# fgiral000/gencast-flax-nnx

Measured on AMD Instinct MI355X. Metric: denoiser-calls/sec, higher is better.
Workload: dtype f16x3 (every product = 3 fp16 MFMAs on hi/lo-split f32 operands: 22-bit products, f32 accumulate; f32 storage); 1 GPU; nano-GenCast DPM-Solver++2S 20-step sample, 2.5deg grid (73x144), 1 ensemble member per GPU, batch 1; dead_call_skipped=True, grid_nodes=10512, mesh_nodes=2562, latent=256, layers=16, heads=4, ffw_hidden=2048, c_in=262, c_out=82, k_hop=8, parallelism=ensemble-dp1, broadcast=none, rccl_ranks=0, precision=f16x3, library_built_from_this_tree=True, launcher=single

## Files before the change

gencast-flax-nnx_amd/csrc/gc_api.hip:

```cpp
#include <dlfcn.h>

#include "gc_handle.h"

using namespace gci;

namespace {

void protect_pending_noise(gc_handle* h) {
  if (h->guard_pending && h->d_noise == h->last_noise) std::swap(h->d_noise, h->d_noise_alt);
}

int check_ready(gc_handle* h) {
  if (!h) return GC_ERR_INVALID_ARGUMENT;
  if (!h->finalized) return fail(h, GC_ERR_STATE, "gc_finalize has not been called");
  return GC_OK;
}

struct Rccl {
  void* lib = nullptr;
  ncclResult_t (*GetUniqueId)(ncclUniqueId*) = nullptr;
  ncclResult_t (*CommInitRank)(ncclComm_t*, int, ncclUniqueId, int) = nullptr;
  ncclResult_t (*CommDestroy)(ncclComm_t) = nullptr;
  ncclResult_t (*CommCount)(const ncclComm_t, int*) = nullptr;
  ncclResult_t (*CommUserRank)(const ncclComm_t, int*) = nullptr;
// ... 67 lines not shown
  if (!out || cap < 16 || device_id < 0 || device_id >= gc_device_count()) return GC_ERR_INVALID_ARGUMENT;
  out[0] = 0;
  return hipDeviceGetPCIBusId(out, (int)cap, device_id) == hipSuccess ? GC_OK : GC_ERR_HIP;
}

const char* gc_last_error(const gc_handle* h) { return h ? h->err.c_str() : g_create_error.c_str(); }

static void read_switches(gc_handle* h) {
  auto is = [](const char* name, const char* value) { const char* v = std::getenv(name); return v && std::string(v) == value; };
  auto off = [](const char* name) { const char* v = std::getenv(name); return v && *v && std::atoi(v) == 0; };
  auto on = [](const char* name) { const char* v = std::getenv(name); return v && *v == '1'; };
  h->f16x3 = !is("GC_PRECISION", "f32");
  h->use_graphs = !is("GC_TUNE_GRAPH", "0");
  h->m2g_fuse_sum = !off("GC_TUNE_M2G_FUSE_SUM");
  h->embed_cache = !off("GC_TUNE_EMBED_CACHE");
  h->attn_items = !off("GC_TUNE_ATTN_ITEMS");
  h->mlp_pair = !off("GC_TUNE_MLP_PAIR");
  h->a16 = !off("GC_TUNE_A16");
  h->graph_serialize = on("GC_TUNE_GRAPH_SERIALIZE");
  h->graph_verbose = on("GC_TUNE_GRAPH_VERBOSE");
}

int gc_create(const gc_config* cfg, int device_id, gc_handle** out) {
  return guarded(nullptr, [&]() -> int {
  if (!cfg || !out) { g_create_error = "null argument"; return GC_ERR_INVALID_ARGUMENT; }
  *out = nullptr;
  const gc_config& c = *cfg;
  auto bad = [&](const char* m) { g_create_error = m; return GC_ERR_INVALID_ARGUMENT; };
  if (c.latent_size <= 0 || c.d_model <= 0 || c.num_heads <= 0 || c.ffw_hidden <= 0 ||
      c.num_layers < 0 || c.c_in <= 0 || c.c_out <= 0 || c.batch <= 0)
// ... 683 lines not shown

int gc_get_counter(gc_handle* h, const char* name, int64_t* value) {
  return guarded(h, [&]() -> int {
  if (!h) return GC_ERR_INVALID_ARGUMENT;
  if (!name || !value) return fail(h, GC_ERR_INVALID_ARGUMENT, "null argument");
  const std::string n(name);
  if (n == "range_fallbacks") *value = h->range_fallbacks;
  else if (n == "static_embedding_fallbacks") *value = h->static_embedding_fallbacks;
  else if (n == "launches_per_call") *value = h->launches_last_call;
  else if (n == "weights_f16_unsafe") *value = h->weights_f16_unsafe ? 1 : 0;
  else if (n == "fp16_storage") *value = h->last_route.st16 ? 1 : 0;
  else if (n == "split_edge") *value = h->split_edge ? 1 : 0;
  else if (n == "attention_items") *value = h->last_route.att_items;
  else if (n == "m2g_fused_sum") *value = h->last_route.m2g_fused ? 1 : 0;
  else if (n == "embed_cache") *value = h->embed_cache_samples;
  else if (n == "graph_replays") *value = h->graph_replays;
  else if (n == "graph_captures") *value = h->graph_captures;
  else if (n == "loss_evaluations") *value = h->loss_evaluations;
  else if (n == "loss_device_us") *value = h->loss_device_us;
  else if (n == "ens_scores") *value = h->ens_scores;
  else if (n == "ens_score_device_us") *value = h->ens_score_device_us;
  else if (n == "ens_invalid_points") *value = h->ens_invalid_points;
  else if (n == "spec_calls") *value = h->spec_calls;
  else if (n == "spec_device_us") *value = h->spec_device_us;
  else if (n == "spec_invalid_columns") *value = h->spec_invalid_columns;
  else if (n == "ens_event_calls") *value = h->evt_calls;
  else if (n == "ens_event_device_us") *value = h->evt_device_us;
  else if (n == "ens_event_invalid_points") *value = h->evt_invalid_points;
  else if (n == "ens_derive_calls") *value = h->drv_calls;
  else if (n == "ens_derive_device_us") *value = h->drv_device_us;
// ... 374 lines not shown
  });
}

int gc_debug_fetch(gc_handle* h, const char* name, float* out, int64_t capacity, int64_t* rows,
                   int64_t* cols) {
  return guarded(h, [&]() -> int {
  int rc = check_ready(h);
  if (rc) return rc;
  if (!name || !rows || !cols) return fail(h, GC_ERR_INVALID_ARGUMENT, "null argument");
  const gc_config& c = h->cfg;
  const gc::HostGraph& g = h->hg;
  const int64_t B = c.batch, L = c.latent_size;
  struct Ent { const char* n; const float* p; int64_t items; int64_t w; int mesh; int batched; int act; };
  const Ent table[] = {
      {"cond", h->d_condvec, 1, gc::kCondDim, 0, 1, 0},
      {"g0", h->d_g0, g.G, L, 0, 1, 1},        {"m0", h->d_m0, g.M, L, 1, 1, 1},
      {"e1", h->d_e1, g.E1, L, 0, 1, 1},       {"agg1", h->d_agg1, g.M, L, 1, 1, 1},
      {"m1", h->d_x, g.M, L, 1, 1, 1},         {"x", h->d_x, g.M, L, 1, 1, 1},
      {"g1", h->d_g1, g.G, L, 0, 1, 1},        {"qkv", h->d_qkv, g.M, 3 * L, 1, 1, 0},
      {"att", h->d_att, g.M, L, 1, 1, 1},      {"m2", h->d_m2, g.M, L, 1, 1, 1},
      {"h", h->d_h, g.M, L, 1, 1, 1},
      {"f1", h->d_f1, g.E2, L, 0, 1, 1},       {"agg2", h->d_agg2, g.G, L, 0, 1, 1},
      {"g2", h->d_g2, g.G, L, 0, 1, 1},        {"y", h->d_y, g.G, c.c_out, 0, 1, 0},
      {"m0_hat", h->d_m0_hat, g.M, L, 1, 0, 0}, {"e0_hat", h->d_e0_hat, g.E1, L, 0, 0, 0},
      {"f0_hat", h->d_f0_hat, g.E2, L, 0, 0, 0},
  };
  if (!std::strncmp(name, "cond:", 5)) {
    auto it = h->cond_sites.find(name + 5);
    if (it == h->cond_sites.end()) return fail(h, GC_ERR_INVALID_ARGUMENT, std::string("unknown conditioning site: ") + (name + 5));
    const int off = it->second.first, w = it->second.second;
    *rows = B;
// ... 123 lines not shown
```

gencast-flax-nnx_amd/csrc/gc_forward.hip:

```cpp
#include "gc_handle.h"

namespace gci {

template <class To, class From>
static const To& a16_view(const From& v) {
  static_assert(sizeof(To) == sizeof(From), "argument struct mismatch between the two kernel builds");
  return reinterpret_cast<const To&>(v);
}

Route make_route(const gc_handle* h) {
  const int D = h->cfg.d_model, F = h->cfg.ffw_hidden;
  Route r;
  r.f16 = h->f16x3 && !h->weights_f16_unsafe && !h->in_fallback;
  r.x32 = !r.f16 && h->f32_ws;
  const bool streams = r.f16 || r.x32;
  r.ffw_slabs = streams ? h->ffw_fused_slabs : 0;
  r.st16 = h->feat16 && h->a16 && r.f16 && D % 128 == 0 && D <= 512 &&
           (h->ffw_fused_slabs > 0 || (F % 128 == 0 && (F / h->ffw2_splits) % 128 == 0));
  r.v2 = r.f16 && r.ws(3 * D, D, 1);
  r.att_items = (h->att_n_items > 0 && r.ws(3 * D, D, 1) && h->attn_splits == 1 && D <= 512) ? h->att_n_items : 0;
  r.fuse_row = streams && D % 128 == 0 && D <= 512;
  r.node_ws = r.f16;
  r.split_edge = h->split_edge;
  r.try_pair = h->mlp_pair && h->hidden_layers == 1;
  r.m2g_fused = h->m2g_fuse_sum && h->hg.m2g_tri && h->hidden_layers == 1 && streams;
  r.embed_cache = h->embed_cache_live && h->embed_cache_ready && !h->feat16 && h->hidden_layers == 1 && streams;
  return r;
}

static gc::Segment seg(const float* ptr, const int* index, const float* affine, int width, int ld, int bcast) {
  gc::Segment s;
  s.ptr = ptr; s.index = index; s.affine = affine; s.width = width; s.ld = ld; s.bcast = bcast;
  return s;
}

struct MlpCall {
  gc::Segment seg[3] = {};
  gc::AddTerm add[2] = {};
  int nseg = 0, nadd = 0, rows = 0, B = 1, ldo = 0;
  bool ln = true, cond = true;
  const float* residual = nullptr;
  float* out = nullptr;
  bool round_out = true;
  bool seg0_f32 = false, out_f32 = false;
  bool tri = false;
  MlpCall& segments(std::initializer_list<gc::Segment> l) { for (const auto& s : l) seg[nseg++] = s; return *this; }
  MlpCall& add_terms(std::initializer_list<gc::AddTerm> l) { for (const auto& t : l) add[nadd++] = t; return *this; }
};
static MlpCall mlp_call(std::initializer_list<gc::Segment> segs, int rows, int B, float* out, int ldo,
                        const float* residual = nullptr) {
  MlpCall c;
  c.rows = rows; c.B = B; c.out = out; c.ldo = ldo; c.residual = residual;
  return c.segments(segs);
}

static int build_mlp_args(gc_handle* h, const DevMlp& w, const MlpCall& c, gc::MlpArgs* out_args) {
  const Route& r = h->route;
  gc::MlpArgs& a = *out_args;
  a = gc::MlpArgs{};
  a.nseg = c.nseg; a.nadd = c.nadd;
  std::copy(c.seg, c.seg + c.nseg, a.seg);
  std::copy(c.add, c.add + c.nadd, a.add);
  a.rows = c.rows; a.B = c.B; a.hidden = h->cfg.latent_size;
  a.f16 = r.f16 ? 1 : 0;
  const Weight& w1 = c.nadd ? w.w1e : w.w1;
  a.w1t = pick(w1, r, Form::Staged); a.ldw1 = w1.ld; a.b1 = w.b1;
  a.w2t = pick(w.w2, r, Form::Staged); a.b2 = w.b2;
  if (r.f16 || r.x32) {
    a.w1f = pick(w1, r, Form::Streaming); a.k1f = w1.kf;
    a.w2f = pick(w.w2, r, Form::Streaming); a.ones = h->d_ones; a.zeros = h->d_zeros;
    a.f32w = r.x32 ? 1 : 0;
  }
  a.n_out = w.n_out; a.n_out_pad = w.n_out_pad; a.do_ln = c.ln ? 1 : 0;
  a.cond = (c.cond && w.cond_off >= 0) ? (h->cond_cur ? h->cond_cur : h->d_cond) + w.cond_off : nullptr;
  a.cond_stride = h->cond_total;
  a.residual = c.residual; a.out = c.out; a.ldo = c.ldo;
  a.round16 = h->feat16 ? 1 : 0;
  a.round_out = (h->feat16 && c.round_out) ? 1 : 0;
  a.a16 = r.st16 ? 1 : 0;
  a.seg0_f32 = c.seg0_f32 ? 1 : 0;
// ... 123 lines not shown
  ga.round16 = 0;
  ga.out_f32 = 1;
  if (r.node_ws) {
    ga.wt = pick(w, r, Form::Streaming); ga.a16 = r.st16 ? 1 : 0;
    return enqueue_gemm_ws(h, gc::KC_GEMM_NODE, ga, pick_ws_mt(rows, L, 1), 1, 0);
  }
  ga.wt = pick(w, r, Form::Staged);
  return launch(h, gc::KC_GEMM_NODE, [&] { return gc::launch_gemm(h->stream, gc::KC_GEMM_NODE, ga, 1, 0, r.f16); });
}
static int edge_node_products(gc_handle* h, const DevMlp& w, const float* senders, int snd_rows, float* snd_out,
                              const float* receivers, int rcv_rows, float* rcv_out) {
  if (int rc = node_gemm(h, senders, snd_rows, w.w1snd, snd_out)) return rc;
  return node_gemm(h, receivers, rcv_rows, w.w1rcv, rcv_out);
}

static MlpCall edge_call(gc_handle* h, const float* e_hat, const float* e_affine, int E, const int* snd, const int* rcv,
                         const float* nsnd, const float* nrcv, const float* psnd, const float* prcv, float* out) {
  const int B = h->cfg.batch, L = h->cfg.latent_size;
  MlpCall c = mlp_call({seg(e_hat, nullptr, e_affine, L, L, 1)}, E * B, B, out, L);
  c.seg0_f32 = true;
  if (h->route.split_edge) c.add_terms({{psnd, snd}, {prcv, rcv}});
  else c.segments({seg(nsnd, snd, nullptr, L, L, 0), seg(nrcv, rcv, nullptr, L, L, 0)});
  return c;
}

int run_m2g_edge(gc_handle* h, const float* cond, bool fused) {
  MlpCall c = edge_call(h, h->d_f0_hat, cond + h->m2g_embed_edge.cond_off, h->hg.E2, h->d_m2g_snd, h->d_m2g_rcv,
                        h->d_m2, h->d_g1, h->d_pm, h->d_pg, fused ? h->d_agg2 : h->d_f1);
  c.tri = fused;
  return run_mlp(h, h->m2g_edge, c);
// ... 11 lines not shown
  if (h->attn_splits > 1) ga->att_S = h->attn_splits;
  else ga->att_tiles = h->d_att_tiles;
}
static int mesh_gemm(gc_handle* h, int cls, const float* a, int lda, const Weight& w, int n, int k, int splits,
                     const float* bias, int act, float* out, int ldo, int epi, bool att_merge = false) {
  const Route& r = h->route;
  const bool ws = r.ws(n, k, splits);
  gc::GemmArgs ga = mesh_gemm_args(h, a, lda, ws);
  ga.wt = pick(w, r, ws ? Form::Streaming : Form::Staged); ga.ldw = k; ga.n = n; ga.k_slice = k / splits;
  ga.bias = bias; ga.act = act; ga.out = out; ga.ldo = ldo;
  if (att_merge) merge_attention_partials(h, &ga);
  if (ws) return enqueue_gemm_ws(h, cls, ga, att_merge ? 1 : pick_ws_mt(ga.rows, n, splits), splits, epi);
  return launch(h, cls, [&] { return gc::launch_gemm(h->stream, cls, ga, splits, epi, r.f16); });
}

int forward(gc_handle* h, float sigma_scalar, const float* cond_ready) {
  const gc_config& c = h->cfg;
  const gc::HostGraph& g = h->hg;
  const int B = c.batch, L = c.latent_size, D = c.d_model, F = c.ffw_hidden;
  hipStream_t s = h->stream;
  int rc;
  const float* cond = cond_ready ? cond_ready : h->d_cond;
  h->cond_cur = cond;
  const int cs = h->cond_total;
  const int64_t launches0 = h->launch_count;
  const Route& r = h->route = h->last_route = make_route(h);

  if (!cond_ready && (rc = launch(h, gc::KC_COND, [&] {
         return gc::launch_cond(s, sigma_scalar < 0 ? h->d_sigma : nullptr, sigma_scalar, B, h->d_nw0t,
                                h->d_nb0, h->d_nw1t, h->d_nb1, c.noise_num_frequencies, c.noise_hidden,
                                c.noise_base_period, h->d_wc_all, h->d_bc_all, cs, h->d_condvec,
                                h->d_cond);
       })))
    return rc;

  {
    MlpCall embed = r.embed_cache ? mlp_call({seg(h->d_xn, nullptr, nullptr, h->nwp, h->nwp, 0)}, g.G * B, B, h->d_g0, L)
                                  : mlp_call({seg(h->d_xp, nullptr, nullptr, h->kp, h->kp, 0)}, g.G * B, B, h->d_g0, L);
    embed.seg0_f32 = true;
    if (r.embed_cache) embed.add_terms({{h->d_pstat, nullptr}});
    if ((rc = run_mlp(h, r.embed_cache ? h->g2m_embed_grid_n : h->g2m_embed_grid, embed))) return rc;
  }
  if ((rc = launch(h, gc::KC_PACK, [&] {
         return gc::launch_affine_rows(s, h->d_m0_hat, cond + h->g2m_embed_mesh.cond_off, cs, g.M, B, L,
                                       h->d_m0, h->feat16, r.st16);
       })))
    return rc;
  const MlpCall edge = edge_call(h, h->d_e0_hat, cond + h->g2m_embed_edge.cond_off, g.E1, h->d_g2m_snd, h->d_g2m_rcv,
                                 h->d_g0, h->d_m0, h->d_pg, h->d_pm, h->d_e1);
  const MlpCall node = mlp_call({seg(h->d_g0, nullptr, nullptr, L, L, 0)}, g.G * B, B, h->d_g1, L, h->d_g0);
  gc::MlpArgs ea{}, na{};
  bool paired = false;
  if (r.try_pair) {
    if ((rc = build_mlp_args(h, h->g2m_edge, edge, &ea)) || (rc = build_mlp_args(h, h->g2m_grid, node, &na))) return rc;
    paired = gc::mlp_pair_supported(ea, na);
  }
  if (r.split_edge && (rc = edge_node_products(h, h->g2m_edge, h->d_g0, g.G * B, h->d_pg, h->d_m0, g.M * B, h->d_pm)))
    return rc;
  if ((rc = paired ? enqueue_mlp_pair(h, ea, na) : run_mlp(h, h->g2m_edge, edge))) return rc;
  if ((rc = launch(h, gc::KC_SEGSUM, [&] {
         return gc::launch_segsum(s, h->d_e1, h->d_g2m_ptr, h->d_g2m_eid, g.M, g.E1, B, L, h->d_agg1, h->feat16, r.st16,
                                  h->g2m_agg_norm);
       })))
    return rc;
  if ((rc = run_mlp(h, h->g2m_mesh, mlp_call({seg(h->d_m0, nullptr, nullptr, L, L, 0), seg(h->d_agg1, nullptr, nullptr, L, L, 0)},
                                             g.M * B, B, h->d_x, L, h->d_m0))))
    return rc;
  if (!paired && (rc = run_mlp(h, h->g2m_grid, node))) return rc;

  const int MB = g.M * B;
  const int n_layers = (h->debug_layer_limit >= 0 && h->debug_layer_limit < c.num_layers)
                           ? h->debug_layer_limit : c.num_layers;
  const float* pend_bias = nullptr;
  int pend_slabs = 0;
  auto rowop = [&](const float* bias, int slabs, int cond_off, float* hout) {
    return launch(h, gc::KC_ROWOP, [&] {
      return gc::launch_rowop(s, h->d_x, bias, h->d_part, slabs, MB, D, B, cond + cond_off, cs, hout, 0, h->feat16, r.st16);
    });
  };
  auto stop_here = [&](int i, int phase) { return h->debug_stop_layer == i && h->debug_stop_phase == phase; };
  const int* att_items = r.att_items ? h->d_att_items : nullptr;
  for (int i = 0; i < n_layers; ++i) {
// ... 108 lines not shown
```

gencast-flax-nnx_amd/csrc/gc_handle.h:

```cpp
#pragma once
#include <hip/hip_runtime.h>

#include <algorithm>
#include <array>
#include <cmath>
#include <cstdio>
#include <cstdlib>
#include <cstring>
#include <map>
#include <memory>
#include <mutex>
#include <string>
#include <vector>

#include <rccl/rccl.h>

#include "../../include/gencast_hip.h"
#include "../../include/gencast_hip_debug.h"
#include "gc_graph.h"
#include "gc_kernels.h"

namespace gci {

inline int round_up(int v, int m) { return (v + m - 1) / m * m; }

struct Route {
  bool f16 = false;
  bool x32 = false;
  bool st16 = false;
  int ffw_slabs = 0;
  bool v2 = false;
  int att_items = 0;
  bool fuse_row = false;
  bool node_ws = false;
  bool m2g_fused = false;
  bool split_edge = false;
  bool try_pair = false;
  bool embed_cache = false;
  bool ws(int n, int k, int splits) const { return (f16 || x32) && n % 128 == 0 && (k / splits) % 128 == 0; }
};

struct Weight {
  float* t = nullptr;
  float* s = nullptr;
  float* f = nullptr;
  float* x = nullptr;
  int ld = 0, kf = 0;
};
enum class Form { Staged, Streaming };
inline const float* pick(const Weight& w, const Route& r, Form form) {
  if (form == Form::Streaming) return r.x32 ? w.x : w.f;
  return r.f16 ? w.s : w.t;
}

struct DevMlp {
  Weight w1, w2;
  Weight w1e, w1snd, w1rcv;
  float *b1 = nullptr, *b2 = nullptr;
  int n_out = 0, n_out_pad = 0;
  int cond_off = -1;
  std::vector<DevMlp> pre;
};

struct DevLayer {
  Weight wqkv, wo, w1, w2;
  float *bo = nullptr, *b1 = nullptr, *b2 = nullptr;
  int cond_attn = -1, cond_ffw = -1;
};

struct BufferGroup {
  std::vector<void*> ptrs;
  explicit BufferGroup(std::vector<BufferGroup*>& of_handle) { of_handle.push_back(this); }
// ... 81 lines not shown
  float *d_feats = nullptr, *d_xp = nullptr, *d_g0 = nullptr, *d_g1 = nullptr, *d_m0 = nullptr,
        *d_x = nullptr, *d_e1 = nullptr, *d_agg1 = nullptr, *d_qkv = nullptr, *d_att = nullptr,
        *d_u = nullptr, *d_m2 = nullptr, *d_f1 = nullptr, *d_agg2 = nullptr, *d_g2 = nullptr,
        *d_y = nullptr, *d_h = nullptr, *d_part = nullptr, *d_apart_o = nullptr, *d_apart_ml = nullptr,
        *d_pg = nullptr, *d_pm = nullptr;
  bool mlp_pair = true;
  bool embed_cache = true;
  bool embed_cache_ready = false;
  bool embed_cache_live = false;
  int nwp = 0;
  float *d_xn = nullptr, *d_pstat = nullptr;
  float *w1st_t = nullptr, *w1st_s = nullptr;
  gci::DevMlp g2m_embed_grid_n;
  std::vector<int> h_slots;
  int64_t embed_cache_samples = 0;
  bool m2g_fuse_sum = true;
  float *d_ones = nullptr, *d_zeros = nullptr;
  int hidden_layers = 1;
  float* d_mlp_tmp[2] = {nullptr, nullptr};
  float *d_feats2 = nullptr, *d_ro_a = nullptr, *d_ro_b = nullptr, *d_ro_forc = nullptr;
  int *d_ro_kind = nullptr, *d_ro_src = nullptr, *d_ro_sidx = nullptr;
  int ro_nforc = -1, ro_forc_cap = 0;
  bool has_sample = false;
  int max_tile_chunks = 0;
  int ffw_fused_slabs = 0;
  void* d_kv16 = nullptr;
  bool f32_ws = true;
  bool split_edge = false;
  int attn_splits = 1, out_splits = 1, ffw2_splits = 1;
  gci::Route route;
// ... 170 lines not shown
  int reg_dev_M = 0;
  int* d_reg_plan = nullptr;
  double* d_reg_part = nullptr;
  unsigned* d_reg_hpart = nullptr;
  double* d_reg_sums = nullptr;
  unsigned long long* d_reg_hist = nullptr;
  gci::Bracket reg_time{events};
  int64_t reg_calls = 0, reg_device_us = 0, reg_invalid_points = 0;

  struct SampleGraph {
    std::vector<float> sigmas;
    int skip_dead = 1;
    const float* noise = nullptr;
    bool feat16 = false;
    gci::Route route;
    hipGraph_t graph = nullptr;
    hipGraphExec_t exec = nullptr, exec2 = nullptr;
    hipEvent_t done[2] = {nullptr, nullptr};
    int next = 0;
    int calls = 0;
    int64_t launches_per_call = 0, launches = 0;
    uint64_t last_use = 0;
  };
  bool use_graphs = true;
  std::vector<SampleGraph> sample_graphs;
  uint64_t graph_clock = 0;
  int64_t graph_replays = 0, graph_captures = 0;
  int debug_layer_limit = -1;
  int debug_stop_layer = -1, debug_stop_phase = -1;
  bool f16x3 = true;
// ... 112 lines not shown
  }
  try {
    (h ? h->err : g_create_error) = what;
  } catch (...) {
  }
  return GC_ERR_INTERNAL;
}

extern const char* const P_M2G;
void build_specs(gc_handle* h);
float f16_bits_to_f32(uint16_t h);
void free_weights(gc_handle* h);
int finalize_weights(gc_handle* h);
int build_embed_cache(gc_handle* h);
Route make_route(const gc_handle* h);
bool build_attention_items(const gc::HostGraph& g, std::vector<int>* items, std::vector<int>* tiles);
int run_m2g_edge(gc_handle* h, const float* cond, bool fused);
int forward(gc_handle* h, float sigma_scalar, const float* cond_ready = nullptr);
int compute_static_embeddings(gc_handle* h);
int guard_enqueue(gc_handle* h, const float* p, size_t n);
bool guard_tripped(gc_handle* h);
int noise_field(gc_handle* h, const float* base, float scale, float* out);
int run_sampler(gc_handle* h, const float* sigmas, int n, int skip_dead, gc_sample_stats* stats);
int resolve_guard(gc_handle* h);
void destroy_sample_graph(gc_handle::SampleGraph& g);
void drop_sample_graphs(gc_handle* h);
int loss_eval(gc_handle* h, int e, const float* sig, bool draw_noise, bool want_den);

}
```

gencast-flax-nnx_amd/csrc/gc_kernels.hip:

```cpp
#include "gc_kernels.h"

#include <algorithm>
#include <atomic>
#include <type_traits>

#include <math.h>
#include <stdlib.h>

#ifdef GC_TU_A16
#define GC_TU_NS gc_a16
#else
#define GC_TU_NS gc
#endif
namespace GC_TU_NS {
#ifdef GC_TU_A16
constexpr bool kTuA16 = true;
#else
constexpr bool kTuA16 = false;
#endif

#include "gc_dev_common.inc"


struct DynLdsOnce {
// ... 3443 lines not shown
__global__ __launch_bounds__(256) void gc_dpm_second_kernel(const float* __restrict__ y,
                                                             const float* __restrict__ xmid,
                                                             float c_out, float c_skip, float a_next,
                                                             size_t n, float* __restrict__ x, NoisyWrite nw) {
  for (size_t i = (size_t)blockIdx.x * 256 + threadIdx.x; i < n; i += (size_t)gridDim.x * 256) {
    const float md = y[i] * c_out + xmid[i] * c_skip;
    const float v = a_next * x[i] + (1.0f - a_next) * md;
    x[i] = v;
    if (nw.xp || nw.xn) put_noisy(nw, i, v);
  }
}

__global__ __launch_bounds__(256) void gc_affine_rows_kernel(const float* __restrict__ src,
                                                              const float* __restrict__ cond,
                                                              int cond_stride, size_t items, int B,
                                                              int w, float* __restrict__ out, int round16, int h16) {
  const size_t total = items * B * w;
  for (size_t i = (size_t)blockIdx.x * 256 + threadIdx.x; i < total; i += (size_t)gridDim.x * 256) {
    const size_t row = i / w;
    const int c = (int)(i - row * w);
    const size_t item = row / B;
    const int b = (int)(row - item * B);
    const float* cs = cond + (size_t)b * cond_stride;
    const float v = src[item * w + c] * cs[c] + cs[w + c];
    if (h16) as_h16(out)[i] = (_Float16)v;
    else out[i] = r16_if(v, round16);
  }
}

static int ew_grid(size_t n) {
  size_t g = (n + 255) / 256;
  return (int)(g > 2048 ? 2048 : (g ? g : 1));
}

hipError_t launch_pack_full(hipStream_t s, const float* grid_struct, const float* feats, int G, int B,
                            int c_in, int kp, float* xp) {
  hipLaunchKernelGGL(gc_pack_full_kernel, dim3(ew_grid((size_t)G * B * kp)), dim3(256), 0, s,
                     grid_struct, feats, G, B, c_in, kp, xp);
  return hipGetLastError();
}

// ... 4 lines not shown
  return hipGetLastError();
}

hipError_t launch_write_noisy_compact(hipStream_t s, const float* x, int rows, int c_out, int ldn, float scale, float* xn) {
  hipLaunchKernelGGL(gc_write_noisy_compact_kernel, dim3(ew_grid((size_t)rows * c_out)), dim3(256), 0, s, x, rows, c_out, ldn,
                     scale, xn);
  return hipGetLastError();
}

hipError_t launch_zero_slots(hipStream_t s, const int* slots, int rows, int c_out, int kp, float* xp) {
  hipLaunchKernelGGL(gc_zero_slots_kernel, dim3(ew_grid((size_t)rows * c_out)), dim3(256), 0, s, slots, rows, c_out, kp, xp);
  return hipGetLastError();
}

hipError_t launch_affine_rows(hipStream_t s, const float* src, const float* cond, int cond_stride,
                              int items, int B, int w, float* out, bool round16, bool h16) {
  hipLaunchKernelGGL(gc_affine_rows_kernel, dim3(ew_grid((size_t)items * B * w)), dim3(256), 0, s, src,
                     cond, cond_stride, (size_t)items, B, w, out, round16 ? 1 : 0, h16 ? 1 : 0);
  return hipGetLastError();
}

hipError_t launch_scale(hipStream_t s, const float* src, float a, size_t n, float* dst, const NoisyWrite& nw) {
  hipLaunchKernelGGL(gc_scale_kernel, dim3(ew_grid(n)), dim3(256), 0, s, src, a, n, dst, nw);
  return hipGetLastError();
}

hipError_t launch_dpm_first(hipStream_t s, const float* y, const float* x, float c_out, float c_skip,
                            float a_mid, size_t n, float* den, float* mid, const NoisyWrite& nw) {
  hipLaunchKernelGGL(gc_dpm_first_kernel, dim3(ew_grid(n)), dim3(256), 0, s, y, x, c_out, c_skip,
                     a_mid, n, den, mid, nw);
  return hipGetLastError();
}

// ... 187 lines not shown
```

gencast-flax-nnx_amd/csrc/gc_kernels_decl.inc:

```
namespace GC_KERNELS_NS {

enum KernelClass : int {
  KC_COND = 0,
  KC_PACK,
  KC_MLP,
  KC_SEGSUM,
  KC_ROWOP,
  KC_GEMM_QKV,
  KC_ATTN,
  KC_ATTN_COMBINE,
  KC_GEMM_OUT,
  KC_GEMM_FFW1,
  KC_GEMM_FFW2,
  KC_GEMM_NODE,
  KC_NOISE,
  KC_COUNT
};

constexpr int kTileM = 32;
constexpr int kCondDim = 16;

struct Segment {
  const float* ptr;
  const int* index;
// ... 142 lines not shown
                               bool h16 = false ,
                               const int* items = nullptr ,
                               int n_items = 0);
#ifdef GC_STAMPS
hipError_t set_attention_stamp_buffer(unsigned long long* p);
#endif

hipError_t launch_pack_full(hipStream_t s, const float* grid_struct, const float* feats, int G, int B,
                            int c_in, int kp, float* xp);
hipError_t launch_write_noisy(hipStream_t s, const float* x, const int* slots, int rows, int c_out,
                              int kp, float scale, float* xp);
hipError_t launch_write_noisy_compact(hipStream_t s, const float* x, int rows, int c_out, int ldn, float scale, float* xn);
hipError_t launch_zero_slots(hipStream_t s, const int* slots, int rows, int c_out, int kp, float* xp);
hipError_t launch_affine_rows(hipStream_t s, const float* src, const float* cond, int cond_stride,
                              int items, int B, int w, float* out, bool round16 = false,
                              bool h16 = false );
hipError_t launch_finite_check(hipStream_t s, const float* p, size_t n, unsigned* counter);
constexpr int kItemPieces = 4;
struct NoisyWrite {
  const int* slots = nullptr;
  int c_out = 1, kp = 0;
  float scale = 0.f;
  float* xp = nullptr;
  float* xn = nullptr;
  int ldn = 0;
  bool active() const { return xp != nullptr || xn != nullptr; }
};
hipError_t launch_scale(hipStream_t s, const float* src, float a, size_t n, float* dst, const NoisyWrite& nw = NoisyWrite());
hipError_t launch_rollout_advance(hipStream_t s, const float* old_feats, const float* sample, const float* forcings,
                                  const int* kind, const int* src, const int* sidx, const float* a, const float* b,
                                  int rows, int c_in, int c_out, int n_forcing, float* new_feats);
// ... 27 lines not shown
```

gencast-flax-nnx_amd/csrc/gc_sampler.hip:

```cpp
#include "gc_handle.h"

namespace gci {

int guard_enqueue(gc_handle* h, const float* p, size_t n) {
  if (!make_route(h).f16) return GC_OK;
  int rc = launch(h, gc::KC_PACK, [&] { return gc::launch_finite_check(h->stream, p, n, h->d_nonfinite); });
  if (rc) return rc;
  GC_HIP(h, hipMemcpyAsync(h->h_nonfinite, h->d_nonfinite, sizeof(unsigned), hipMemcpyDeviceToHost, h->stream));
  return GC_OK;
}
bool guard_tripped(gc_handle* h) {
  if (*h->h_nonfinite == h->nonfinite_seen) return false;
  h->nonfinite_seen = *h->h_nonfinite;
  return true;
}

float f_c_in(float s) { return 1.0f / std::sqrt(s * s + 1.0f); }
float f_c_out(float s) { return s / std::sqrt(s * s + 1.0f); }
float f_c_skip(float s) { return 1.0f / (s * s + 1.0f); }

int noise_field(gc_handle* h, const float* base, float scale, float* out) {
  if (h->nz_L == 0) return fail(h, GC_ERR_STATE, "gc_noise_set_tables has not been called");
  const int N = h->cfg.batch * h->cfg.c_out;
  const size_t ncoef = (size_t)2 * h->nz_L * h->nz_L * N;
// ... 4 lines not shown
    return gc::launch_noise_synthesis(h->stream, h->d_nz_leg, h->d_nz_cos, h->d_nz_sin, h->d_nz_coef, h->d_nz_f,
                                      h->nz_L, h->nz_lat, h->nz_lon, N, base, scale, out);
  });
}

int sampler_body(gc_handle* h, const float* sigmas, int n, int skip_dead, const std::vector<float>& call_sigma,
                 bool multi, int* calls_out) {
  const gc_config& c = h->cfg;
  const int rows = h->hg.G * c.batch;
  const size_t ne = (size_t)rows * c.c_out;
  hipStream_t s = h->stream;
  int rc, calls = 0;
  const size_t cond_call = (size_t)c.batch * h->cond_total;
  const bool churn = !h->churn_rates.empty();
  h->embed_cache_live = true;
  struct CacheOff { gc_handle* h; ~CacheOff() { h->embed_cache_live = false; } } cache_off{h};
  const Route route = make_route(h);
  const bool cache = route.embed_cache;
  if (cache) {
    if ((rc = launch(h, gc::KC_PACK, [&] { return gc::launch_zero_slots(s, h->d_slots, rows, c.c_out, h->kp, h->d_xp); }))) return rc;
    gc::GemmArgs ga{};
    ga.a = h->d_xp; ga.lda = h->kp; ga.a_f32 = 1; ga.ldw = h->kp; ga.rows = rows; ga.n = c.latent_size; ga.k_slice = h->kp;
    ga.bias = nullptr; ga.act = 0; ga.out = h->d_pstat; ga.ldo = c.latent_size; ga.round16 = 0; ga.out_f32 = 1;
    ga.wt = route.f16 ? h->w1st_s : h->w1st_t;
    if ((rc = launch(h, gc::KC_GEMM_NODE, [&] { return gc::launch_gemm(s, gc::KC_GEMM_NODE, ga, 1, 0, route.f16); }))) return rc;
    ++h->embed_cache_samples;
  }
  auto noisy_write = [&](float sigma_next_call) {
    gc::NoisyWrite nw;
    nw.slots = h->d_slots; nw.c_out = c.c_out; nw.kp = h->kp; nw.scale = f_c_in(std::max(sigma_next_call, 1e-6f));
    if (cache) { nw.xn = h->d_xn; nw.ldn = h->nwp; }
// ... 6 lines not shown
    const gc::NoisyWrite nw = (n > 0 && !churned(0)) ? noisy_write(sigmas[0]) : gc::NoisyWrite();
    if ((rc = launch(h, gc::KC_PACK, [&] { return gc::launch_scale(s, h->d_noise, sigmas[0], ne, h->d_sx, nw); })))
      return rc;
    written = nw.active();
  }
  if (multi) {
    gc::SigmaList sl{};
    for (size_t i = 0; i < call_sigma.size(); ++i) sl.v[i] = call_sigma[i];
    if ((rc = launch(h, gc::KC_COND, [&] {
           return gc::launch_cond_multi(s, sl, (int)call_sigma.size(), c.batch, h->d_nw0t, h->d_nb0, h->d_nw1t,
                                        h->d_nb1, c.noise_num_frequencies, c.noise_hidden, c.noise_base_period,
                                        h->d_wc_all, h->d_bc_all, h->cond_total, h->d_cond_all);
         })))
      return rc;
  }
  auto denoise = [&](const float* x, float sigma) -> int {
    const float ss = std::max(sigma, 1e-6f);
    if (!written) {
      int r = launch(h, gc::KC_PACK, [&] {
        return cache ? gc::launch_write_noisy_compact(s, x, rows, c.c_out, h->nwp, f_c_in(ss), h->d_xn)
                     : gc::launch_write_noisy(s, x, h->d_slots, rows, c.c_out, h->kp, f_c_in(ss), h->d_xp);
      });
      if (r) return r;
    }
    written = false;
    const float* ready = nullptr;
    if (multi) {
      if (calls >= (int)call_sigma.size() || call_sigma[calls] != ss)
        return fail(h, GC_ERR_INTERNAL, "sampler: noise-level list out of step with the loop");
      ready = h->d_cond_all + (size_t)calls * cond_call;
    }
    ++calls;
    return forward(h, ss, ready);
  };
  for (int i = 0; i < n; ++i) {
    float sg = sigmas[i];
    const float sn = sigmas[i + 1];
    if (churn && h->churn_rates[i] > 0.f) {
      const float s_new = sg * (1.0f + h->churn_rates[i]);
      const float extra = std::sqrt(std::max(s_new * s_new - sg * sg, 0.0f)) * h->churn_inflation;
      if ((rc = noise_field(h, h->d_sx, extra, h->d_sx))) return rc;
      sg = s_new;
    }
    const float sm = std::sqrt(sg * sn);
    if ((rc = denoise(h->d_sx, sg))) return rc;
    const float ss = std::max(sg, 1e-6f);
    const float a_mid = sm / sg;
    {
// ... 39 lines not shown
  if (churn && (int)h->churn_rates.size() != n)
    return fail(h, GC_ERR_INVALID_ARGUMENT, "gc_set_churn was given a schedule of another length than this sample");
  std::vector<float> call_sigma;
  for (int i = 0; i < n; ++i) {
    float sg = sigmas[i];
    if (churn && h->churn_rates[i] > 0.f) sg = sg * (1.0f + h->churn_rates[i]);
    call_sigma.push_back(std::max(sg, 1e-6f));
    const float sn = sigmas[i + 1];
    if (sn != 0.0f || !skip_dead) call_sigma.push_back(std::max(std::sqrt(sg * sn), 1e-6f));
  }
  const bool multi = (int)call_sigma.size() <= gc::kMaxSigmaList;
  const size_t cond_call = (size_t)c.batch * h->cond_total;
  if (multi && call_sigma.size() * cond_call > h->cond_all_cap) {
    if ((rc = dev_alloc(h, &h->d_cond_all, call_sigma.size() * cond_call))) return rc;
    h->cond_all_cap = call_sigma.size() * cond_call;
  }

  const bool eligible = h->use_graphs && multi && !churn && h->prof_cls < 0 && h->debug_layer_limit < 0 &&
                        h->debug_stop_layer < 0;
  gc_handle::SampleGraph* sg = nullptr;
  if (eligible) {
    const Route r = make_route(h);
    for (auto& g : h->sample_graphs)
      if (g.skip_dead == skip_dead && g.noise == h->d_noise && g.route.f16 == r.f16 && g.feat16 == h->feat16 && g.route.st16 == r.st16 &&
          (int)g.sigmas.size() == n + 1 && !std::memcmp(g.sigmas.data(), sigmas, (n + 1) * sizeof(float)))
        sg = &g;
    if (!sg) {
      if (h->sample_graphs.size() >= 8) {
        size_t lru = 0;
        for (size_t i = 1; i < h->sample_graphs.size(); ++i)
// ... 18 lines not shown
    if (h->graph_serialize) launch_lock.lock();
    const int i = g->exec2 ? g->next : 0;
    hipGraphExec_t ex = i ? g->exec2 : g->exec;
    if (!g->done[i]) GC_HIP(h, hipEventCreateWithFlags(&g->done[i], hipEventDisableTiming));
    else GC_HIP(h, hipEventSynchronize(g->done[i]));
    GC_HIP(h, hipGraphLaunch(ex, s));
    GC_HIP(h, hipEventRecord(g->done[i], s));
    g->next = i ^ 1;
    return GC_OK;
  };
  if (sg && sg->exec) {
    if ((rc = launch_exec(sg))) return rc;
    calls = sg->calls;
    h->launches_last_call = sg->launches_per_call;
    h->route = h->last_route = sg->route;
    ++h->graph_replays;
  } else if (sg) {
    const int64_t l0 = h->launch_count;
    auto say = [&](const char* what) { if (h->graph_verbose) { std::fprintf(stderr, "[gc graph] %s\n", what); std::fflush(stderr); } };
    hipGraph_t graph = nullptr;
    hipGraphExec_t exec = nullptr, exec2 = nullptr;
    {
      std::lock_guard<std::mutex> capture_lock(capture_mutex);
      say("begin capture");
      GC_HIP(h, hipStreamBeginCapture(s, hipStreamCaptureModeThreadLocal));
      rc = sampler_body(h, sigmas, n, skip_dead, call_sigma, multi, &calls);
      const hipError_t e_end = hipStreamEndCapture(s, &graph);
      say("end capture");
      if (rc) {
        if (graph) (void)hipGraphDestroy(graph);
// ... 1 lines not shown
      }
      if (e_end != hipSuccess || !graph) return fail(h, GC_ERR_HIP, std::string("hipStreamEndCapture: ") + hipGetErrorString(e_end));
      hipError_t e_inst = hipGraphInstantiate(&exec, graph, nullptr, nullptr, 0);
      if (e_inst == hipSuccess) e_inst = hipGraphInstantiate(&exec2, graph, nullptr, nullptr, 0);
      if (e_inst != hipSuccess) {
        if (exec) (void)hipGraphExecDestroy(exec);
        (void)hipGraphDestroy(graph);
        return fail(h, GC_ERR_HIP, std::string("hipGraphInstantiate: ") + hipGetErrorString(e_inst));
      }
      say("instantiated");
    }
    sg->graph = graph; sg->exec = exec; sg->exec2 = exec2; sg->calls = calls; sg->next = 0;
    sg->launches = h->launch_count - l0;
    sg->launches_per_call = h->launches_last_call;
    sg->route = h->last_route;
    ++h->graph_captures;
    if ((rc = launch_exec(sg))) return rc;
    say("launched");
    ++h->graph_replays;
  } else if ((rc = sampler_body(h, sigmas, n, skip_dead, call_sigma, multi, &calls))) {
    return rc;
  }
  GC_HIP(h, hipEventRecord(h->ev1, s));
  h->has_sample = true;
  if (make_route(h).f16) {
    if ((rc = guard_enqueue(h, h->d_sx, ne))) return rc;
    h->last_sigmas.assign(sigmas, sigmas + n + 1);
    h->last_skip_dead = skip_dead;
    h->guard_pending = true;
    h->last_stream0 = stream0;
// ... 79 lines not shown
```

gencast-flax-nnx_amd/csrc/gc_weights.hip:

```cpp
#include "gc_handle.h"

namespace gci {

const char* const P_NOISE = "denoiser.noise_level_encoder";
const char* const P_G2M = "denoiser.predictor.grid2mesh_gnn";
const char* const P_M2G = "denoiser.predictor.mesh2grid_gnn";
const char* const P_TR = "denoiser.predictor.mesh_gnn.batch_first_transformer";

void add_mlp_specs(gc_handle* h, const std::string& p, int n_in, int n_hid, int n_out, bool cond) {
  const int nh = h->hidden_layers;
  for (int i = 0; i < nh; ++i) {
    const std::string l = p + ".network.network.layers." + std::to_string(2 * i);
    h->specs[l + ".kernel"] = {i == 0 ? n_in : n_hid, n_hid};
    h->specs[l + ".bias"] = {n_hid};
  }
  const std::string l = p + ".network.network.layers." + std::to_string(2 * nh);
  h->specs[l + ".kernel"] = {n_hid, n_out};
  h->specs[l + ".bias"] = {n_out};
  if (cond) {
    h->specs[p + ".norm_conditioning_layer.conditional_linear_layer.kernel"] = {gc::kCondDim, 2 * n_out};
    h->specs[p + ".norm_conditioning_layer.conditional_linear_layer.bias"] = {2 * n_out};
  }
}

// ... 329 lines not shown
    for (int i = 0; i < gc::kCondDim; ++i)
      for (int j = 0; j < 2 * cdim; ++j) wc[(size_t)i * cp.total + off + j] = k[(size_t)i * 2 * cdim + j];
    for (int j = 0; j < 2 * cdim; ++j) bc[off + j] = b[j] + (j < cdim ? 1.0f : 0.0f);
    off += 2 * cdim;
  }
  if ((rc = dev_upload(h, &h->d_wc_all, wc, own))) return rc;
  if ((rc = dev_upload(h, &h->d_bc_all, bc, own))) return rc;
  if ((rc = dev_alloc(h, &h->d_cond, (size_t)c.batch * cp.total, own))) return rc;

  const int nf2 = 2 * c.noise_num_frequencies;
  if ((rc = dev_upload(h, &h->d_nw0t, transpose_pad(h->weights.at(nz + ".linear_0.kernel"), nf2, c.noise_hidden, 0, nf2, nf2, c.noise_hidden), own))) return rc;
  if ((rc = dev_upload(h, &h->d_nb0, h->weights.at(nz + ".linear_0.bias"), own))) return rc;
  if ((rc = dev_upload(h, &h->d_nw1t, transpose_pad(h->weights.at(nz + ".linear_1.kernel"), c.noise_hidden, gc::kCondDim, 0, c.noise_hidden, c.noise_hidden, gc::kCondDim), own))) return rc;
  if ((rc = dev_upload(h, &h->d_nb1, h->weights.at(nz + ".linear_1.bias"), own))) return rc;

  h->weights_f16_unsafe = false;
  for (const auto& kv : h->weights)
    for (float w : kv.second)
      if (!(std::fabs(w) <= 65504.0f)) { h->weights_f16_unsafe = true; break; }
  if ((rc = compute_static_embeddings(h))) return rc;
  h->finalized = true;
  h->finalized_weights = true;
  return build_embed_cache(h);
}

}
```

Before: 763.0 calls/s.

## Precompute per-noise-level mesh embeddings and their first-layer products for all sampler calls

Adds a sigma cache. Before the sampler runs, one batched pass builds, for every denoiser call in the sample, the conditioned mesh-node embedding `m0` and its products with the receiver slice of the grid2mesh edge MLP's first-layer weights and the m0 slice of the mesh-node MLP's first-layer weights. Each forward then reads these slices instead of running the affine pack. The edge and mesh MLPs run with narrower first-layer weights (2L and L inputs instead of 3L and 2L) plus an add-term. This moves per-call per-edge and per-node GEMM work into one larger batched GEMM per sample, at the cost of extra device memory under a budget. A vectorized affine-rows kernel is also added.

```diff
diff --git a/gencast-flax-nnx_amd/csrc/gc_api.hip b/gencast-flax-nnx_amd/csrc/gc_api.hip
--- a/gencast-flax-nnx_amd/csrc/gc_api.hip
+++ b/gencast-flax-nnx_amd/csrc/gc_api.hip
@@ -105,6 +105,9 @@
   h->use_graphs = !is("GC_TUNE_GRAPH", "0");
   h->m2g_fuse_sum = !off("GC_TUNE_M2G_FUSE_SUM");
   h->embed_cache = !off("GC_TUNE_EMBED_CACHE");
+  h->sigma_cache = !off("GC_TUNE_SIGMA_CACHE");
+  if (const char* mb = std::getenv("GC_TUNE_SIGMA_CACHE_MB"))
+    if (*mb) h->sigma_cache_budget = (size_t)std::max(0L, std::atol(mb)) << 20;
   h->attn_items = !off("GC_TUNE_ATTN_ITEMS");
   h->mlp_pair = !off("GC_TUNE_MLP_PAIR");
   h->a16 = !off("GC_TUNE_A16");
@@ -818,6 +821,8 @@
   else if (n == "attention_items") *value = h->last_route.att_items;
   else if (n == "m2g_fused_sum") *value = h->last_route.m2g_fused ? 1 : 0;
   else if (n == "embed_cache") *value = h->embed_cache_samples;
+  else if (n == "sigma_cache") *value = h->last_route.sigma_cache ? 1 : 0;
+  else if (n == "sigma_cache_samples") *value = h->sigma_cache_samples;
   else if (n == "graph_replays") *value = h->graph_replays;
   else if (n == "graph_captures") *value = h->graph_captures;
   else if (n == "loss_evaluations") *value = h->loss_evaluations;
@@ -1222,7 +1227,7 @@
   struct Ent { const char* n; const float* p; int64_t items; int64_t w; int mesh; int batched; int act; };
   const Ent table[] = {
       {"cond", h->d_condvec, 1, gc::kCondDim, 0, 1, 0},
-      {"g0", h->d_g0, g.G, L, 0, 1, 1},        {"m0", h->d_m0, g.M, L, 1, 1, 1},
+      {"g0", h->d_g0, g.G, L, 0, 1, 1},        {"m0", h->m0_cur ? h->m0_cur : h->d_m0, g.M, L, 1, 1, 1},
       {"e1", h->d_e1, g.E1, L, 0, 1, 1},       {"agg1", h->d_agg1, g.M, L, 1, 1, 1},
       {"m1", h->d_x, g.M, L, 1, 1, 1},         {"x", h->d_x, g.M, L, 1, 1, 1},
       {"g1", h->d_g1, g.G, L, 0, 1, 1},        {"qkv", h->d_qkv, g.M, 3 * L, 1, 1, 0},
diff --git a/gencast-flax-nnx_amd/csrc/gc_forward.hip b/gencast-flax-nnx_amd/csrc/gc_forward.hip
--- a/gencast-flax-nnx_amd/csrc/gc_forward.hip
+++ b/gencast-flax-nnx_amd/csrc/gc_forward.hip
@@ -6,6 +6,11 @@
 static const To& a16_view(const From& v) {
   static_assert(sizeof(To) == sizeof(From), "argument struct mismatch between the two kernel builds");
   return reinterpret_cast<const To&>(v);
+}
+
+bool sigma_cache_shapes(const gc_handle* h) {
+  const int L = h->cfg.latent_size;
+  return h->hidden_layers == 1 && !h->split_edge && (L == 128 || L == 256) && h->g2m_edge.w1x.f && h->g2m_mesh.w1x.f;
 }
 
 Route make_route(const gc_handle* h) {
@@ -25,6 +30,7 @@
   r.try_pair = h->mlp_pair && h->hidden_layers == 1;
   r.m2g_fused = h->m2g_fuse_sum && h->hg.m2g_tri && h->hidden_layers == 1 && streams;
   r.embed_cache = h->embed_cache_live && h->embed_cache_ready && !h->feat16 && h->hidden_layers == 1 && streams;
+  r.sigma_cache = h->sigma_cache_live && sigma_cache_shapes(h) && streams && !h->in_fallback;
   return r;
 }
 
@@ -44,6 +50,7 @@
   bool round_out = true;
   bool seg0_f32 = false, out_f32 = false;
   bool tri = false;
+  const Weight* w1 = nullptr;
   MlpCall& segments(std::initializer_list<gc::Segment> l) { for (const auto& s : l) seg[nseg++] = s; return *this; }
   MlpCall& add_terms(std::initializer_list<gc::AddTerm> l) { for (const auto& t : l) add[nadd++] = t; return *this; }
 };
@@ -63,7 +70,7 @@
   std::copy(c.add, c.add + c.nadd, a.add);
   a.rows = c.rows; a.B = c.B; a.hidden = h->cfg.latent_size;
   a.f16 = r.f16 ? 1 : 0;
-  const Weight& w1 = c.nadd ? w.w1e : w.w1;
+  const Weight& w1 = c.w1 ? *c.w1 : c.nadd ? w.w1e : w.w1;
   a.w1t = pick(w1, r, Form::Staged); a.ldw1 = w1.ld; a.b1 = w.b1;
   a.w2t = pick(w.w2, r, Form::Staged); a.b2 = w.b2;
   if (r.f16 || r.x32) {
@@ -217,6 +224,19 @@
   return node_gemm(h, receivers, rcv_rows, w.w1rcv, rcv_out);
 }
 
+int build_sigma_tables(gc_handle* h, const float* cond_all, int calls) {
+  const int B = h->cfg.batch, L = h->cfg.latent_size, M = h->hg.M;
+  const Route& r = h->route = make_route(h);
+  if (calls > h->sigma_cap) return fail(h, GC_ERR_INTERNAL, "sigma cache: the tables hold fewer calls than the sample makes");
+  if (int rc = launch(h, gc::KC_PACK, [&] {
+        return gc::launch_affine_rows(h->stream, h->d_m0_hat, cond_all + h->g2m_embed_mesh.cond_off, h->cond_total, M, B, L,
+                                      h->d_sig_m0, h->feat16, r.st16, calls);
+      }))
+    return rc;
+  if (int rc = node_gemm(h, h->d_sig_m0, calls * M * B, h->g2m_edge.w1rcv, h->d_sig_pmr)) return rc;
+  return node_gemm(h, h->d_sig_m0, calls * M * B, h->g2m_mesh.w1m0, h->d_sig_pmn);
+}
+
 static MlpCall edge_call(gc_handle* h, const float* e_hat, const float* e_affine, int E, const int* snd, const int* rcv,
                          const float* nsnd, const float* nrcv, const float* psnd, const float* prcv, float* out) {
   const int B = h->cfg.batch, L = h->cfg.latent_size;
@@ -258,7 +278,7 @@
   return launch(h, cls, [&] { return gc::launch_gemm(h->stream, cls, ga, splits, epi, r.f16); });
 }
 
-int forward(gc_handle* h, float sigma_scalar, const float* cond_ready) {
+int forward(gc_handle* h, float sigma_scalar, const float* cond_ready, int call) {
   const gc_config& c = h->cfg;
   const gc::HostGraph& g = h->hg;
   const int B = c.batch, L = c.latent_size, D = c.d_model, F = c.ffw_hidden;
@@ -269,6 +289,15 @@
   const int cs = h->cond_total;
   const int64_t launches0 = h->launch_count;
   const Route& r = h->route = h->last_route = make_route(h);
+  if (r.sigma_cache && (call < 0 || call >= h->sigma_cap || !cond_ready))
+    return fail(h, GC_ERR_INTERNAL, "sigma cache: a forward outside the sample's noise-level list");
+  const size_t sig_slice = (size_t)g.M * B * L;
+  const float* m0 = r.sigma_cache ? (r.st16 ? reinterpret_cast<const float*>(reinterpret_cast<const _Float16*>(h->d_sig_m0) + call * sig_slice)
+                                            : h->d_sig_m0 + call * sig_slice)
+                                  : h->d_m0;
+  const float* pmr = r.sigma_cache ? h->d_sig_pmr + call * sig_slice : nullptr;
+  const float* pmn = r.sigma_cache ? h->d_sig_pmn + call * sig_slice : nullptr;
+  h->m0_cur = m0;
 
   if (!cond_ready && (rc = launch(h, gc::KC_COND, [&] {
          return gc::launch_cond(s, sigma_scalar < 0 ? h->d_sigma : nullptr, sigma_scalar, B, h->d_nw0t,
@@ -285,13 +314,18 @@
     if (r.embed_cache) embed.add_terms({{h->d_pstat, nullptr}});
     if ((rc = run_mlp(h, r.embed_cache ? h->g2m_embed_grid_n : h->g2m_embed_grid, embed))) return rc;
   }
-  if ((rc = launch(h, gc::KC_PACK, [&] {
+  if (!r.sigma_cache && (rc = launch(h, gc::KC_PACK, [&] {
          return gc::launch_affine_rows(s, h->d_m0_hat, cond + h->g2m_embed_mesh.cond_off, cs, g.M, B, L,
                                        h->d_m0, h->feat16, r.st16);
        })))
     return rc;
-  const MlpCall edge = edge_call(h, h->d_e0_hat, cond + h->g2m_embed_edge.cond_off, g.E1, h->d_g2m_snd, h->d_g2m_rcv,
-                                 h->d_g0, h->d_m0, h->d_pg, h->d_pm, h->d_e1);
+  MlpCall edge = edge_call(h, h->d_e0_hat, cond + h->g2m_embed_edge.cond_off, g.E1, h->d_g2m_snd, h->d_g2m_rcv,
+                           h->d_g0, m0, h->d_pg, h->d_pm, h->d_e1);
+  if (r.sigma_cache) {
+    edge.nseg = 2;
+    edge.add_terms({{pmr, h->d_g2m_rcv}});
+    edge.w1 = &h->g2m_edge.w1x;
+  }
   const MlpCall node = mlp_call({seg(h->d_g0, nullptr, nullptr, L, L, 0)}, g.G * B, B, h->d_g1, L, h->d_g0);
   gc::MlpArgs ea{}, na{};
   bool paired = false;
@@ -299,7 +333,7 @@
     if ((rc = build_mlp_args(h, h->g2m_edge, edge, &ea)) || (rc = build_mlp_args(h, h->g2m_grid, node, &na))) return rc;
     paired = gc::mlp_pair_supported(ea, na);
   }
-  if (r.split_edge && (rc = edge_node_products(h, h->g2m_edge, h->d_g0, g.G * B, h->d_pg, h->d_m0, g.M * B, h->d_pm)))
+  if (r.split_edge && (rc = edge_node_products(h, h->g2m_edge, h->d_g0, g.G * B, h->d_pg, m0, g.M * B, h->d_pm)))
     return rc;
   if ((rc = paired ? enqueue_mlp_pair(h, ea, na) : run_mlp(h, h->g2m_edge, edge))) return rc;
   if ((rc = launch(h, gc::KC_SEGSUM, [&] {
@@ -307,9 +341,13 @@
                                   h->g2m_agg_norm);
        })))
     return rc;
-  if ((rc = run_mlp(h, h->g2m_mesh, mlp_call({seg(h->d_m0, nullptr, nullptr, L, L, 0), seg(h->d_agg1, nullptr, nullptr, L, L, 0)},
-                                             g.M * B, B, h->d_x, L, h->d_m0))))
-    return rc;
+  MlpCall mesh = mlp_call({seg(m0, nullptr, nullptr, L, L, 0), seg(h->d_agg1, nullptr, nullptr, L, L, 0)}, g.M * B, B, h->d_x, L, m0);
+  if (r.sigma_cache) {
+    mesh = mlp_call({seg(h->d_agg1, nullptr, nullptr, L, L, 0)}, g.M * B, B, h->d_x, L, m0);
+    mesh.add_terms({{pmn, nullptr}});
+    mesh.w1 = &h->g2m_mesh.w1x;
+  }
+  if ((rc = run_mlp(h, h->g2m_mesh, mesh))) return rc;
   if (!paired && (rc = run_mlp(h, h->g2m_grid, node))) return rc;
 
   const int MB = g.M * B;
diff --git a/gencast-flax-nnx_amd/csrc/gc_handle.h b/gencast-flax-nnx_amd/csrc/gc_handle.h
--- a/gencast-flax-nnx_amd/csrc/gc_handle.h
+++ b/gencast-flax-nnx_amd/csrc/gc_handle.h
@@ -37,6 +37,7 @@
   bool split_edge = false;
   bool try_pair = false;
   bool embed_cache = false;
+  bool sigma_cache = false;
   bool ws(int n, int k, int splits) const { return (f16 || x32) && n % 128 == 0 && (k / splits) % 128 == 0; }
 };
 
@@ -56,6 +57,7 @@
 struct DevMlp {
   Weight w1, w2;
   Weight w1e, w1snd, w1rcv;
+  Weight w1x, w1m0;
   float *b1 = nullptr, *b2 = nullptr;
   int n_out = 0, n_out_pad = 0;
   int cond_off = -1;
@@ -167,6 +169,15 @@
   gci::DevMlp g2m_embed_grid_n;
   std::vector<int> h_slots;
   int64_t embed_cache_samples = 0;
+  bool sigma_cache = true;
+  size_t sigma_cache_budget = (size_t)1 << 30;
+  bool sigma_cache_live = false;
+  gci::BufferGroup sigma_allocs{groups};
+  int sigma_cap = 0;
+  size_t sigma_held = 0;
+  float *d_sig_m0 = nullptr, *d_sig_pmr = nullptr, *d_sig_pmn = nullptr;
+  const float* m0_cur = nullptr;
+  int64_t sigma_cache_samples = 0;
   bool m2g_fuse_sum = true;
   float *d_ones = nullptr, *d_zeros = nullptr;
   int hidden_layers = 1;
@@ -367,6 +378,7 @@
     const float* noise = nullptr;
     bool feat16 = false;
     gci::Route route;
+    const float* m0_last = nullptr;
     hipGraph_t graph = nullptr;
     hipGraphExec_t exec = nullptr, exec2 = nullptr;
     hipEvent_t done[2] = {nullptr, nullptr};
@@ -509,10 +521,12 @@
 int finalize_weights(gc_handle* h);
 int build_embed_cache(gc_handle* h);
 Route make_route(const gc_handle* h);
+bool sigma_cache_shapes(const gc_handle* h);
 bool build_attention_items(const gc::HostGraph& g, std::vector<int>* items, std::vector<int>* tiles);
 int run_m2g_edge(gc_handle* h, const float* cond, bool fused);
-int forward(gc_handle* h, float sigma_scalar, const float* cond_ready = nullptr);
+int forward(gc_handle* h, float sigma_scalar, const float* cond_ready = nullptr, int call = -1);
 int compute_static_embeddings(gc_handle* h);
+int build_sigma_tables(gc_handle* h, const float* cond_all, int calls);
 int guard_enqueue(gc_handle* h, const float* p, size_t n);
 bool guard_tripped(gc_handle* h);
 int noise_field(gc_handle* h, const float* base, float scale, float* out);
diff --git a/gencast-flax-nnx_amd/csrc/gc_kernels.hip b/gencast-flax-nnx_amd/csrc/gc_kernels.hip
--- a/gencast-flax-nnx_amd/csrc/gc_kernels.hip
+++ b/gencast-flax-nnx_amd/csrc/gc_kernels.hip
@@ -3481,17 +3481,41 @@
 __global__ __launch_bounds__(256) void gc_affine_rows_kernel(const float* __restrict__ src,
                                                               const float* __restrict__ cond,
                                                               int cond_stride, size_t items, int B,
-                                                              int w, float* __restrict__ out, int round16, int h16) {
-  const size_t total = items * B * w;
+                                                              int w, float* __restrict__ out, int round16, int h16,
+                                                              int calls) {
+  const size_t per_call = items * B, total = per_call * calls * w;
   for (size_t i = (size_t)blockIdx.x * 256 + threadIdx.x; i < total; i += (size_t)gridDim.x * 256) {
-    const size_t row = i / w;
-    const int c = (int)(i - row * w);
+    const size_t row_all = i / w;
+    const int c = (int)(i - row_all * w);
+    const size_t call = row_all / per_call, row = row_all - call * per_call;
     const size_t item = row / B;
     const int b = (int)(row - item * B);
-    const float* cs = cond + (size_t)b * cond_stride;
+    const float* cs = cond + (call * B + b) * cond_stride;
     const float v = src[item * w + c] * cs[c] + cs[w + c];
     if (h16) as_h16(out)[i] = (_Float16)v;
     else out[i] = r16_if(v, round16);
+  }
+}
+__global__ __launch_bounds__(256) void gc_affine_rows4_kernel(const float* __restrict__ src,
+                                                               const float* __restrict__ cond,
+                                                               int cond_stride, size_t items, int B,
+                                                               int w, float* __restrict__ out, int round16, int h16,
+                                                               int calls) {
+  const int w4 = w >> 2;
+  const size_t per_call = items * B, total = per_call * calls * w4;
+  for (size_t i = (size_t)blockIdx.x * 256 + threadIdx.x; i < total; i += (size_t)gridDim.x * 256) {
+    const size_t row_all = i / w4;
+    const int c = (int)(i - row_all * w4) * 4;
+    const size_t call = row_all / per_call, row = row_all - call * per_call;
+    const size_t item = row / B;
+    const int b = (int)(row - item * B);
+    const float* cs = cond + (call * B + b) * cond_stride;
+    const f32x4 x = ld4(src + item * w + c), sc = ld4(cs + c), of = ld4(cs + w + c);
+    f32x4 v;
+#pragma unroll
+    for (int e = 0; e < 4; ++e) v[e] = x[e] * sc[e] + of[e];
+    if (h16) sth4(as_h16(out) + row_all * w + c, v);
+    else st4(out + row_all * w + c, r16_if(v, round16));
   }
 }
 
@@ -3526,9 +3550,16 @@
 }
 
 hipError_t launch_affine_rows(hipStream_t s, const float* src, const float* cond, int cond_stride,
-                              int items, int B, int w, float* out, bool round16, bool h16) {
-  hipLaunchKernelGGL(gc_affine_rows_kernel, dim3(ew_grid((size_t)items * B * w)), dim3(256), 0, s, src,
-                     cond, cond_stride, (size_t)items, B, w, out, round16 ? 1 : 0, h16 ? 1 : 0);
+                              int items, int B, int w, float* out, bool round16, bool h16, int calls) {
+  if (calls < 1) return hipErrorInvalidValue;
+  const auto al16 = [](const void* p) { return (reinterpret_cast<size_t>(p) & 15) == 0; };
+  if (w % 4 == 0 && cond_stride % 4 == 0 && al16(src) && al16(cond) && al16(out)) {
+    hipLaunchKernelGGL(gc_affine_rows4_kernel, dim3(ew_grid((size_t)calls * items * B * (w / 4))), dim3(256), 0, s, src,
+                       cond, cond_stride, (size_t)items, B, w, out, round16 ? 1 : 0, h16 ? 1 : 0, calls);
+    return hipGetLastError();
+  }
+  hipLaunchKernelGGL(gc_affine_rows_kernel, dim3(ew_grid((size_t)calls * items * B * w)), dim3(256), 0, s, src,
+                     cond, cond_stride, (size_t)items, B, w, out, round16 ? 1 : 0, h16 ? 1 : 0, calls);
   return hipGetLastError();
 }
 
diff --git a/gencast-flax-nnx_amd/csrc/gc_kernels_decl.inc b/gencast-flax-nnx_amd/csrc/gc_kernels_decl.inc
--- a/gencast-flax-nnx_amd/csrc/gc_kernels_decl.inc
+++ b/gencast-flax-nnx_amd/csrc/gc_kernels_decl.inc
@@ -180,7 +180,8 @@
 hipError_t launch_zero_slots(hipStream_t s, const int* slots, int rows, int c_out, int kp, float* xp);
 hipError_t launch_affine_rows(hipStream_t s, const float* src, const float* cond, int cond_stride,
                               int items, int B, int w, float* out, bool round16 = false,
-                              bool h16 = false );
+                              bool h16 = false ,
+                              int calls = 1 );
 hipError_t launch_finite_check(hipStream_t s, const float* p, size_t n, unsigned* counter);
 constexpr int kItemPieces = 4;
 struct NoisyWrite {
diff --git a/gencast-flax-nnx_amd/csrc/gc_sampler.hip b/gencast-flax-nnx_amd/csrc/gc_sampler.hip
--- a/gencast-flax-nnx_amd/csrc/gc_sampler.hip
+++ b/gencast-flax-nnx_amd/csrc/gc_sampler.hip
@@ -42,7 +42,8 @@
   const size_t cond_call = (size_t)c.batch * h->cond_total;
   const bool churn = !h->churn_rates.empty();
   h->embed_cache_live = true;
-  struct CacheOff { gc_handle* h; ~CacheOff() { h->embed_cache_live = false; } } cache_off{h};
+  h->sigma_cache_live = h->sigma_cache && multi && (int)call_sigma.size() <= h->sigma_cap;
+  struct CacheOff { gc_handle* h; ~CacheOff() { h->embed_cache_live = h->sigma_cache_live = false; } } cache_off{h};
   const Route route = make_route(h);
   const bool cache = route.embed_cache;
   if (cache) {
@@ -79,6 +80,10 @@
          })))
       return rc;
   }
+  if (route.sigma_cache) {
+    if ((rc = build_sigma_tables(h, h->d_cond_all, (int)call_sigma.size()))) return rc;
+    ++h->sigma_cache_samples;
+  }
   auto denoise = [&](const float* x, float sigma) -> int {
     const float ss = std::max(sigma, 1e-6f);
     if (!written) {
@@ -96,7 +101,7 @@
       ready = h->d_cond_all + (size_t)calls * cond_call;
     }
     ++calls;
-    return forward(h, ss, ready);
+    return forward(h, ss, ready, multi ? calls - 1 : -1);
   };
   for (int i = 0; i < n; ++i) {
     float sg = sigmas[i];
@@ -166,6 +171,27 @@
   if (multi && call_sigma.size() * cond_call > h->cond_all_cap) {
     if ((rc = dev_alloc(h, &h->d_cond_all, call_sigma.size() * cond_call))) return rc;
     h->cond_all_cap = call_sigma.size() * cond_call;
+  }
+  const int ncalls = (int)call_sigma.size();
+  if (h->sigma_cache && multi && !h->in_fallback && sigma_cache_shapes(h) && ncalls > h->sigma_cap) {
+    const size_t slice = (size_t)h->hg.M * c.batch * c.latent_size, bytes = 3 * ncalls * slice * sizeof(float);
+    if (bytes <= h->sigma_cache_budget) {
+      if (h->sigma_held + bytes > h->sigma_cache_budget) {
+        drop_sample_graphs(h);
+        GC_HIP(h, h->sigma_allocs.drop(s));
+        h->sigma_held = 0;
+      }
+      h->sigma_cap = 0;
+      if (dev_alloc(h, &h->d_sig_m0, ncalls * slice, &h->sigma_allocs) == GC_OK &&
+          dev_alloc(h, &h->d_sig_pmr, ncalls * slice, &h->sigma_allocs) == GC_OK &&
+          dev_alloc(h, &h->d_sig_pmn, ncalls * slice, &h->sigma_allocs) == GC_OK) {
+        h->sigma_cap = ncalls;
+        h->sigma_held += bytes;
+      } else {
+        (void)hipGetLastError();
+        h->err.clear();
+      }
+    }
   }
 
   const bool eligible = h->use_graphs && multi && !churn && h->prof_cls < 0 && h->debug_layer_limit < 0 &&
@@ -214,6 +240,7 @@
     calls = sg->calls;
     h->launches_last_call = sg->launches_per_call;
     h->route = h->last_route = sg->route;
+    h->m0_cur = sg->m0_last;
     ++h->graph_replays;
   } else if (sg) {
     const int64_t l0 = h->launch_count;
@@ -245,6 +272,7 @@
     sg->launches = h->launch_count - l0;
     sg->launches_per_call = h->launches_last_call;
     sg->route = h->last_route;
+    sg->m0_last = h->m0_cur;
     ++h->graph_captures;
     if ((rc = launch_exec(sg))) return rc;
     say("launched");
diff --git a/gencast-flax-nnx_amd/csrc/gc_weights.hip b/gencast-flax-nnx_amd/csrc/gc_weights.hip
--- a/gencast-flax-nnx_amd/csrc/gc_weights.hip
+++ b/gencast-flax-nnx_amd/csrc/gc_weights.hip
@@ -367,6 +367,14 @@
   if ((rc = dev_upload(h, &h->d_nw1t, transpose_pad(h->weights.at(nz + ".linear_1.kernel"), c.noise_hidden, gc::kCondDim, 0, c.noise_hidden, c.noise_hidden, gc::kCondDim), own))) return rc;
   if ((rc = dev_upload(h, &h->d_nb1, h->weights.at(nz + ".linear_1.bias"), own))) return rc;
 
+  if (h->hidden_layers == 1) {
+    const auto& ke = h->weights.at(gn + ".update_edge_fns.grid2mesh.edge_fn.network.network.layers.0.kernel");
+    const auto& kn = h->weights.at(gn + ".update_node_fns.mesh_nodes.node_fn.network.network.layers.0.kernel");
+    if ((rc = upload_weight(h, transpose_pad(ke, 3 * L, L, 0, 2 * L, 2 * L, L), L, 2 * L, round_up(2 * L, 64), h->f32_ws, &h->g2m_edge.w1x))) return rc;
+    if ((rc = upload_weight(h, transpose_pad(kn, 2 * L, L, L, L, L, L), L, L, round_up(L, 64), h->f32_ws, &h->g2m_mesh.w1x))) return rc;
+    if ((rc = upload_weight(h, transpose_pad(kn, 2 * L, L, 0, L, L, L), L, L, L, false, &h->g2m_mesh.w1m0))) return rc;
+  }
+
   h->weights_f16_unsafe = false;
   for (const auto& kv : h->weights)
     for (float w : kv.second)
```

Measured after the change: 759.5 calls/s. About the same (-0.5%).
